# meyer-lab/cmtf-pls

Measured on AMD Instinct MI355X. Metric: nipals_iters_per_sec, higher is better.
Workload: dtype f32

## Files before the change

### cmtf_pls_amd/csrc/xcov.hip

```cpp
#include "common.hpp"

namespace cmtfpls {

typedef double d4_t __attribute__((ext_vector_type(4)));

void launch_reduce_rows(const double* part, int nrows, int64_t P, double* out, hipStream_t st);

XcovPlan plan_xcov(int64_t I, int64_t P) {
  XcovPlan p;
  p.col_tiles = (int)((P + 255) / 256);
#ifndef CMTFPLS_XCOV_BLOCKS
#define CMTFPLS_XCOV_BLOCKS 1024
#endif
  int64_t want = (CMTFPLS_XCOV_BLOCKS + p.col_tiles - 1) / p.col_tiles;
  if (want < 1) want = 1;
  int64_t rpb = (I + want - 1) / want;
  rpb = (rpb + 63) / 64 * 64;
  if (rpb < 64) rpb = 64;
  p.rows_per_block = (int)rpb;
  p.row_blocks = (int)((I + rpb - 1) / rpb);
  if (p.row_blocks < 1) p.row_blocks = 1;
  return p;
}

template <typename T, bool MASKED, bool VEC, int MT, bool FAST, bool SSQ = false, bool STATS = false>
__global__ __launch_bounds__(256) void xcov_kernel(const T* __restrict__ X, int64_t I, int64_t P,
                                                  const double* __restrict__ Y, int ldy, int M,
                                                  double* __restrict__ part, int rows_per_block,
                                                  const double* __restrict__ mean = nullptr, double* __restrict__ ssq_part = nullptr) {
  const int lane = threadIdx.x & 63, wv = threadIdx.x >> 6;
  const int kq = lane >> 4, nn = lane & 15;
  const int64_t cb = ((int64_t)blockIdx.x * 4 + wv) * 64;
  if (cb >= P) {
    if (SSQ && lane == 0) ssq_part[((int64_t)blockIdx.y * gridDim.x + blockIdx.x) * 4 + wv] = 0.0;
    return;
  }
  const int64_t c = cb + 4 * nn;
  const int64_t r0 = (int64_t)blockIdx.y * rows_per_block;
  const int64_t r1 = (r0 + rows_per_block < I) ? r0 + rows_per_block : I;
  using XV = Pack<T, 4>;
  d4_t acc[MT][4];
#pragma unroll
  for (int mt = 0; mt < MT; ++mt)
#pragma unroll
    for (int e = 0; e < 4; ++e) acc[mt][e] = d4_t{0.0, 0.0, 0.0, 0.0};
  bool mok[MT];
#pragma unroll
  for (int mt = 0; mt < MT; ++mt) mok[mt] = (mt * 16 + nn) < M;

#ifndef CMTFPLS_XCOV_UN
#define CMTFPLS_XCOV_UN 4
#endif
  constexpr int UN = CMTFPLS_XCOV_UN;
  const int64_t cc = (c < P) ? c : (VEC ? P - 4 : P - 1);
  int ycol[MT];
#pragma unroll
  for (int mt = 0; mt < MT; ++mt) ycol[mt] = mok[mt] ? mt * 16 + nn : M - 1;
  double mu[SSQ ? 4 : 1], ssq = 0.0;
  double cs[STATS ? 4 : 1] = {}, cq[STATS ? 4 : 1] = {};
  if constexpr (SSQ) {
#pragma unroll
    for (int e = 0; e < 4; ++e) mu[e] = mean[(c + e < P) ? c + e : P - 1];
  }

  auto load_stage = [&](XV (&x)[UN], double (&a)[UN][MT], int64_t r) {
#pragma unroll
    for (int s = 0; s < UN; ++s) {
      const int64_t row = r + 4 * s + kq;
      const int64_t rowc = (FAST || row < r1) ? row : r1 - 1;
      if (VEC) {
        x[s] = ld_stream(reinterpret_cast<const XV*>(X + rowc * P + cc));
      } else {
#pragma unroll
        for (int e = 0; e < 4; ++e) x[s].e[e] = X[rowc * P + ((cc + e < P) ? cc + e : P - 1)];
      }
#pragma unroll
      for (int mt = 0; mt < MT; ++mt) a[s][mt] = Y[rowc * ldy + ycol[mt]];
    }
  };
  auto mma_stage = [&](const XV (&x)[UN], const double (&a)[UN][MT], int64_t r) {
#pragma unroll
    for (int s = 0; s < UN; ++s) {
      const bool rok = FAST || (r + 4 * s + kq) < r1;
#pragma unroll
      for (int e = 0; e < 4; ++e) {
        T xv = x[s].e[e];
        if (MASKED) xv = (xv == xv) ? xv : (T)0;
        const double b = (FAST || (rok && c + e < P)) ? (double)xv : 0.0;
        if constexpr (SSQ) {
          const double dv = (FAST || (rok && c + e < P)) ? b - mu[e] : 0.0;
          ssq = fma(dv, dv, ssq);
        }
        if constexpr (STATS) {
          cs[e] += b;
          cq[e] = fma(b, b, cq[e]);
        }
#pragma unroll
        for (int mt = 0; mt < MT; ++mt)
          acc[mt][e] = __builtin_amdgcn_mfma_f64_16x16x4f64((FAST || (rok && mok[mt])) ? a[s][mt] : 0.0, b, acc[mt][e], 0, 0, 0);
      }
    }
  };

  XV xa[UN], xb[UN];
  double aa[UN][MT], ab[UN][MT];
  load_stage(xa, aa, r0);
  for (int64_t r = r0; r < r1; r += 8 * UN) {
    load_stage(xb, ab, r + 4 * UN);
    mma_stage(xa, aa, r);
    load_stage(xa, aa, (FAST && r + 8 * UN >= r1) ? r : r + 8 * UN);
    mma_stage(xb, ab, r + 4 * UN);
  }
  if constexpr (SSQ) {
    ssq = wave_sum(ssq);
    if (lane == 0) ssq_part[((int64_t)blockIdx.y * gridDim.x + blockIdx.x) * 4 + wv] = ssq;
  }
  if constexpr (STATS) {
    double* srow = ssq_part + (int64_t)blockIdx.y * 2 * P;
#pragma unroll
    for (int e = 0; e < 4; ++e) {
      double v = cs[e], w = cq[e];
      v += __shfl_xor(v, 16, kWave);
      v += __shfl_xor(v, 32, kWave);
      w += __shfl_xor(w, 16, kWave);
      w += __shfl_xor(w, 32, kWave);
      if (kq == 0 && c + e < P) { srow[c + e] = v; srow[P + c + e] = w; }
    }
  }
#pragma unroll
  for (int mt = 0; mt < MT; ++mt)
#pragma unroll
    for (int g = 0; g < 4; ++g) {
      const int m = mt * 16 + kq + 4 * g;
      if (m < M) {
        double* dst = part + ((int64_t)blockIdx.y * M + m) * P + c;
#pragma unroll
        for (int e = 0; e < 4; ++e)
          if (c + e < P) dst[e] = acc[mt][e][g];
      }
    }
}

template <typename T, int MT, bool FAST>
__global__ __launch_bounds__(256) void xcov_deflate_kernel(T* __restrict__ X, int64_t I, int64_t P, int B,
                                                          const double* __restrict__ Y, int ldy, int M,
                                                          double* __restrict__ part, int rows_per_block,
                                                          const double* __restrict__ t, const double* __restrict__ wA,
                                                          const double* __restrict__ wB, double* __restrict__ ssq_part) {
  const int lane = threadIdx.x & 63, wv = threadIdx.x >> 6;
  const int kq = lane >> 4, nn = lane & 15;
  const int64_t cb = ((int64_t)blockIdx.x * 4 + wv) * 64;
  if (cb >= P) {
    if (lane == 0) ssq_part[((int64_t)blockIdx.y * gridDim.x + blockIdx.x) * 4 + wv] = 0.0;
    return;
  }
  const int64_t c = cb + 4 * nn;
  const int64_t r0 = (int64_t)blockIdx.y * rows_per_block;
  const int64_t r1 = (r0 + rows_per_block < I) ? r0 + rows_per_block : I;
  using XV = Pack<T, 4>;
  d4_t acc[MT][4];
#pragma unroll
  for (int mt = 0; mt < MT; ++mt)
#pragma unroll
    for (int e = 0; e < 4; ++e) acc[mt][e] = d4_t{0.0, 0.0, 0.0, 0.0};
  bool mok[MT];
#pragma unroll
  for (int mt = 0; mt < MT; ++mt) mok[mt] = (mt * 16 + nn) < M;
  constexpr int UN = CMTFPLS_XCOV_UN;
  const bool cok = c < P;
  const int64_t cc = cok ? c : P - 4;
  int ycol[MT];
#pragma unroll
  for (int mt = 0; mt < MT; ++mt) ycol[mt] = mok[mt] ? mt * 16 + nn : M - 1;
  double wa[4], wb[4], ssq = 0.0;
#pragma unroll
  for (int e = 0; e < 4; ++e) {
    wa[e] = wA[(cc + e) / B];
    wb[e] = wB[(cc + e) % B];
  }

  auto load_stage = [&](XV (&x)[UN], double (&a)[UN][MT], double (&ts)[UN], int64_t r) {
#pragma unroll
    for (int s = 0; s < UN; ++s) {
      const int64_t row = r + 4 * s + kq;
      const int64_t rowc = (FAST || row < r1) ? row : r1 - 1;
      x[s] = ld_stream(reinterpret_cast<const XV*>(X + rowc * P + cc));
      ts[s] = t[rowc];
#pragma unroll
      for (int mt = 0; mt < MT; ++mt) a[s][mt] = Y[rowc * ldy + ycol[mt]];
    }
  };
  auto mma_stage = [&](XV (&x)[UN], const double (&a)[UN][MT], const double (&ts)[UN], int64_t r) {
#pragma unroll
    for (int s = 0; s < UN; ++s) {
      const int64_t row = r + 4 * s + kq;
      const bool rok = FAST || row < r1;
      const bool ok = rok && (FAST || cok);
#pragma unroll
      for (int e = 0; e < 4; ++e) {
        const double tw = ts[s] * wa[e];
        const T nv = (T)fma(-tw, wb[e], (double)x[s].e[e]);
        x[s].e[e] = nv;
        const double b = (ok && nv == nv) ? (double)nv : 0.0;
        ssq = fma(b, b, ssq);
#pragma unroll
        for (int mt = 0; mt < MT; ++mt)
          acc[mt][e] = __builtin_amdgcn_mfma_f64_16x16x4f64((FAST || (rok && mok[mt])) ? a[s][mt] : 0.0, b, acc[mt][e], 0, 0, 0);
      }
      if (ok) st_stream(reinterpret_cast<XV*>(X + row * P + c), x[s]);
    }
  };

  XV xa[UN], xb[UN];
  double aa[UN][MT], ab[UN][MT], ta[UN], tb[UN];
  load_stage(xa, aa, ta, r0);
  for (int64_t r = r0; r < r1; r += 8 * UN) {
    load_stage(xb, ab, tb, r + 4 * UN);
    mma_stage(xa, aa, ta, r);
    load_stage(xa, aa, ta, (r + 8 * UN >= r1) ? r : r + 8 * UN);
    mma_stage(xb, ab, tb, r + 4 * UN);
  }
  ssq = wave_sum(ssq);
  if (lane == 0) ssq_part[((int64_t)blockIdx.y * gridDim.x + blockIdx.x) * 4 + wv] = ssq;
#pragma unroll
  for (int mt = 0; mt < MT; ++mt)
#pragma unroll
    for (int g = 0; g < 4; ++g) {
      const int m = mt * 16 + kq + 4 * g;
      if (m < M) {
        double* dst = part + ((int64_t)blockIdx.y * M + m) * P + c;
#pragma unroll
        for (int e = 0; e < 4; ++e)
          if (c + e < P) dst[e] = acc[mt][e][g];
      }
    }
}

__global__ __launch_bounds__(256) void quadform_kernel(const double* __restrict__ G, int M, const double* __restrict__ q,
                                                      const double* __restrict__ q_old, double* __restrict__ out) {
  __shared__ double red[16];
  double s = 0.0;
  for (int idx = threadIdx.x; idx < M * M; idx += 256) {
    const int i = idx / M, j = idx - i * M;
    s = fma((q[i] - q_old[i]) * G[idx], (q[j] - q_old[j]), s);
  }
  s = block_sum(s, red);
  if (threadIdx.x == 0) out[0] = s;
}

static size_t xcov_ssq_extra(const XcovPlan& p) { return ((size_t)p.row_blocks * p.col_tiles * 4 * sizeof(double) + 255) / 256 * 256; }

template <typename T>
static int run_xcov_tile(const T* X, int64_t I, int64_t P, const double* Y, int ldy, int M, double* S, int masked,
                         void* ws, size_t ws_bytes, hipStream_t st, const double* mean = nullptr, double* ssq_out = nullptr,
                         double* stats_out = nullptr) {
  const XcovPlan p = plan_xcov(I, P);
  const bool with_ssq = ssq_out != nullptr, with_stats = stats_out != nullptr;
  if (with_ssq && (masked || !mean)) { set_error("xcov_ssq: needs the column means and a block without missing values"); return CMTFPLS_EINVAL; }
  if (with_stats && (masked || with_ssq)) { set_error("xcov_stats: a block without missing values, no second norm"); return CMTFPLS_EINVAL; }
  const size_t need = (size_t)p.row_blocks * M * P * sizeof(double) + (with_ssq ? xcov_ssq_extra(p) : 0) +
                      (with_stats ? (size_t)p.row_blocks * 2 * P * sizeof(double) : 0);
  if (!ws || ws_bytes < need) { set_error("xcov: workspace too small"); return CMTFPLS_EWORKSPACE; }
  const bool vec = (P % 4 == 0) && ((reinterpret_cast<uintptr_t>(X) & (4 * sizeof(T) - 1)) == 0);
  const int mt = (M + 15) / 16;
  double* part = static_cast<double*>(ws);
  const dim3 grid(p.col_tiles, p.row_blocks), block(256);
  const bool fast = vec && (P % 256 == 0) && (M % 16 == 0) && (M / 16 != 3) && (I % p.rows_per_block == 0) &&
                    (p.rows_per_block % (8 * 4) == 0);
  double* ssq_part = (with_ssq || with_stats) ? reinterpret_cast<double*>(static_cast<char*>(ws) + (size_t)p.row_blocks * M * P * sizeof(double)) : nullptr;
#define XL(MSK, VC, MTT, FS) hipLaunchKernelGGL((xcov_kernel<T, MSK, VC, MTT, FS>), grid, block, 0, st, X, I, P, Y, ldy, M, part, p.rows_per_block, (const double*)nullptr, (double*)nullptr)
#define XS(VC, MTT, FS) hipLaunchKernelGGL((xcov_kernel<T, false, VC, MTT, FS, true>), grid, block, 0, st, X, I, P, Y, ldy, M, part, p.rows_per_block, mean, ssq_part)
#define XM(MSK, VC, FS) do { if (mt == 1) XL(MSK, VC, 1, FS); else if (mt == 2) XL(MSK, VC, 2, FS); else XL(MSK, VC, 4, FS); } while (0)
#define XQ(VC, FS) do { if (mt == 1) XS(VC, 1, FS); else if (mt == 2) XS(VC, 2, FS); else XS(VC, 4, FS); } while (0)
#define XT1(VC, MTT, FS) hipLaunchKernelGGL((xcov_kernel<T, false, VC, MTT, FS, false, true>), grid, block, 0, st, X, I, P, Y, ldy, M, part, p.rows_per_block, (const double*)nullptr, ssq_part)
#define XT(VC, FS) do { if (mt == 1) XT1(VC, 1, FS); else if (mt == 2) XT1(VC, 2, FS); else XT1(VC, 4, FS); } while (0)
  if (with_stats)  { if (fast) XT(true, true); else if (vec) XT(true, false); else XT(false, false); }
  else if (with_ssq) { if (fast) XQ(true, true); else if (vec) XQ(true, false); else XQ(false, false); }
  else if (masked) { if (fast) XM(true, true, true); else if (vec) XM(true, true, false); else XM(true, false, false); }
  else             { if (fast) XM(false, true, true); else if (vec) XM(false, true, false); else XM(false, false, false); }
#undef XT
#undef XT1
#undef XQ
#undef XM
#undef XS
#undef XL
  launch_reduce_rows(part, p.row_blocks, (int64_t)M * P, S, st);
  if (with_stats) launch_reduce_rows(ssq_part, p.row_blocks, 2 * P, stats_out, st);
  int rc = check_launch("xcov");
  if (rc == CMTFPLS_OK && with_ssq) rc = cmtfpls_sum_f64(ssq_part, (int64_t)p.row_blocks * p.col_tiles * 4, ssq_out, st);
  return rc;
}

template <typename T>
static int run_xcov(const T* X, int64_t I, int64_t P, const double* Y, int ldy, int M, double* S, int masked,
                    void* ws, size_t ws_bytes, hipStream_t st, const double* mean = nullptr, double* ssq_out = nullptr) {
  if (!X || !Y || !S || I <= 0 || P <= 0 || M <= 0 || ldy < M) { set_error("xcov: bad argument"); return CMTFPLS_EINVAL; }
  for (int lo = 0; lo < M; lo += kXcovMaxResponses) {
    const int mt = (M - lo < kXcovMaxResponses) ? M - lo : kXcovMaxResponses;
    const int rc = run_xcov_tile<T>(X, I, P, Y + lo, ldy, mt, S + (int64_t)lo * P, masked, ws, ws_bytes, st, mean, lo == 0 ? ssq_out : nullptr);
    if (rc != CMTFPLS_OK) return rc;
  }
  return CMTFPLS_OK;
}

template <typename T>
static int run_xcov_deflate(T* X, int64_t I, int A, int B, const double* Y, int ldy, int M, const double* t, const double* wA,
                            const double* wB, double* S, double* ssq, void* ws, size_t ws_bytes, hipStream_t st) {
  if (!X || !Y || !S || !t || !wA || !wB || !ssq || I <= 0 || A <= 0 || B <= 0 || M <= 0 || ldy < M) {
    set_error("xcov_deflate: bad argument");
    return CMTFPLS_EINVAL;
  }
  const int64_t P = (int64_t)A * B;
  if (M > 64 || (P % 4) != 0 || (reinterpret_cast<uintptr_t>(X) & (4 * sizeof(T) - 1)) != 0) {
    set_error("xcov_deflate: M > 64 or rows that are not whole 4-element vectors; deflate, then xcov");
    return CMTFPLS_EUNSUPPORTED;
  }
  const XcovPlan p = plan_xcov(I, P);
  const size_t need = (size_t)p.row_blocks * M * P * sizeof(double) + xcov_ssq_extra(p);
  if (!ws || ws_bytes < need) { set_error("xcov_deflate: workspace too small"); return CMTFPLS_EWORKSPACE; }
  const int mt = (M + 15) / 16;
  double* part = static_cast<double*>(ws);
  double* ssq_part = reinterpret_cast<double*>(static_cast<char*>(ws) + (size_t)p.row_blocks * M * P * sizeof(double));
  const dim3 grid(p.col_tiles, p.row_blocks), block(256);
  const bool fast = (P % 256 == 0) && (M % 16 == 0) && (M / 16 != 3) && (I % p.rows_per_block == 0) && (p.rows_per_block % (8 * 4) == 0);
#define XD(MTT, FS) hipLaunchKernelGGL((xcov_deflate_kernel<T, MTT, FS>), grid, block, 0, st, X, I, P, B, Y, ldy, M, part, p.rows_per_block, t, wA, wB, ssq_part)
  if (fast) { if (mt == 1) XD(1, true); else if (mt == 2) XD(2, true); else XD(4, true); }
  else      { if (mt == 1) XD(1, false); else if (mt == 2) XD(2, false); else XD(4, false); }
#undef XD
  launch_reduce_rows(part, p.row_blocks, (int64_t)M * P, S, st);
  int rc = check_launch("xcov_deflate");
  if (rc == CMTFPLS_OK) rc = cmtfpls_sum_f64(ssq_part, (int64_t)p.row_blocks * p.col_tiles * 4, ssq, st);
  return rc;
}

}

using namespace cmtfpls;

extern "C" {

size_t cmtfpls_xcov_workspace_bytes(int64_t I, int64_t P, int M) {
  if (I <= 0 || P <= 0 || M <= 0) return 0;
  const XcovPlan p = plan_xcov(I, P);
  if (M > kXcovMaxResponses) M = kXcovMaxResponses;
  return (size_t)p.row_blocks * M * P * sizeof(double);
}
int cmtfpls_xcov_f32(const float* X, int64_t I, int64_t P, const double* Y, int ldy, int M, double* S, int masked,
                     void* ws, size_t ws_bytes, void* stream) {
  return run_xcov<float>(X, I, P, Y, ldy, M, S, masked, ws, ws_bytes, (hipStream_t)stream);
}
int cmtfpls_xcov_f64(const double* X, int64_t I, int64_t P, const double* Y, int ldy, int M, double* S, int masked,
                     void* ws, size_t ws_bytes, void* stream) {
  return run_xcov<double>(X, I, P, Y, ldy, M, S, masked, ws, ws_bytes, (hipStream_t)stream);
}
size_t cmtfpls_xcov_ssq_workspace_bytes(int64_t I, int64_t P, int M) {
  if (I <= 0 || P <= 0 || M <= 0) return 0;
  const XcovPlan p = plan_xcov(I, P);
  if (M > kXcovMaxResponses) M = kXcovMaxResponses;
  return (size_t)p.row_blocks * M * P * sizeof(double) + xcov_ssq_extra(p);
}
int cmtfpls_xcov_ssq_f32(const float* X, int64_t I, int64_t P, const double* Y, int ldy, int M, double* S, const double* mean,
                         double* ssq, void* ws, size_t ws_bytes, void* stream) {
  if (!mean || !ssq) { set_error("xcov_ssq: bad argument"); return CMTFPLS_EINVAL; }
  return run_xcov<float>(X, I, P, Y, ldy, M, S, 0, ws, ws_bytes, (hipStream_t)stream, mean, ssq);
}
int cmtfpls_xcov_ssq_f64(const double* X, int64_t I, int64_t P, const double* Y, int ldy, int M, double* S, const double* mean,
                         double* ssq, void* ws, size_t ws_bytes, void* stream) {
  if (!mean || !ssq) { set_error("xcov_ssq: bad argument"); return CMTFPLS_EINVAL; }
  return run_xcov<double>(X, I, P, Y, ldy, M, S, 0, ws, ws_bytes, (hipStream_t)stream, mean, ssq);
}
size_t cmtfpls_xcov_stats_workspace_bytes(int64_t I, int64_t P, int M) {
  if (I <= 0 || P <= 0 || M <= 0 || M > kXcovMaxResponses) return 0;
  const XcovPlan p = plan_xcov(I, P);
  return (size_t)p.row_blocks * ((size_t)M + 2) * P * sizeof(double);
}
int cmtfpls_xcov_stats_f32(const float* X, int64_t I, int64_t P, const double* Y, int ldy, int M, double* S, double* stats,
                           void* ws, size_t ws_bytes, void* stream) {
  if (!X || !Y || !S || !stats || I <= 0 || P <= 0 || M <= 0 || ldy < M) { set_error("xcov_stats: bad argument"); return CMTFPLS_EINVAL; }
  if (M > kXcovMaxResponses) { set_error("xcov_stats: more than 64 responses; use colstats + xcov"); return CMTFPLS_EUNSUPPORTED; }
  return run_xcov_tile<float>(X, I, P, Y, ldy, M, S, 0, ws, ws_bytes, (hipStream_t)stream, nullptr, nullptr, stats);
}
int cmtfpls_xcov_stats_f64(const double* X, int64_t I, int64_t P, const double* Y, int ldy, int M, double* S, double* stats,
                           void* ws, size_t ws_bytes, void* stream) {
  if (!X || !Y || !S || !stats || I <= 0 || P <= 0 || M <= 0 || ldy < M) { set_error("xcov_stats: bad argument"); return CMTFPLS_EINVAL; }
  if (M > kXcovMaxResponses) { set_error("xcov_stats: more than 64 responses; use colstats + xcov"); return CMTFPLS_EUNSUPPORTED; }
  return run_xcov_tile<double>(X, I, P, Y, ldy, M, S, 0, ws, ws_bytes, (hipStream_t)stream, nullptr, nullptr, stats);
}
int cmtfpls_xcov_deflate_f32(float* X, int64_t I, int A, int B, const double* Y, int ldy, int M, const double* t, const double* wA,
                             const double* wB, double* S, double* ssq, void* ws, size_t ws_bytes, void* stream) {
  return run_xcov_deflate<float>(X, I, A, B, Y, ldy, M, t, wA, wB, S, ssq, ws, ws_bytes, (hipStream_t)stream);
}
int cmtfpls_xcov_deflate_f64(double* X, int64_t I, int A, int B, const double* Y, int ldy, int M, const double* t, const double* wA,
                             const double* wB, double* S, double* ssq, void* ws, size_t ws_bytes, void* stream) {
  return run_xcov_deflate<double>(X, I, A, B, Y, ldy, M, t, wA, wB, S, ssq, ws, ws_bytes, (hipStream_t)stream);
}
int cmtfpls_quadform_f64(const double* G, int M, const double* q, const double* q_old, double* out, void* stream) {
  if (!G || !q || !q_old || !out || M <= 0) { set_error("quadform: bad argument"); return CMTFPLS_EINVAL; }
  hipLaunchKernelGGL(quadform_kernel, dim3(1), dim3(256), 0, (hipStream_t)stream, G, M, q, q_old, out);
  return check_launch("quadform");
}

}
```

Before: 762.1.

## Have each wave cover multiple 64-column groups in xcov kernels to reuse Y loads

Result: no change. 761.8 (-0.0%).

```diff
diff --git a/cmtf_pls_amd/csrc/xcov.hip b/cmtf_pls_amd/csrc/xcov.hip
--- a/cmtf_pls_amd/csrc/xcov.hip
+++ b/cmtf_pls_amd/csrc/xcov.hip
@@ -23,86 +23,111 @@
   return p;
 }
 
-template <typename T, bool MASKED, bool VEC, int MT, bool FAST, bool SSQ = false, bool STATS = false>
+constexpr int xcov_groups(int MT) { return MT <= 2 ? 2 : 1; }
+#ifndef CMTFPLS_XCOV_UN
+#define CMTFPLS_XCOV_UN 4
+#endif
+
+template <int G>
+__device__ __forceinline__ void xcov_zero_slots(double* ssq_part, int64_t g0, int ngroups, int lane) {
+  if (lane < G && g0 + lane < ngroups) ssq_part[(int64_t)blockIdx.y * ngroups + g0 + lane] = 0.0;
+}
+
+template <typename T, bool MASKED, bool VEC, int MT, int G, bool FAST, bool SSQ = false, bool STATS = false>
 __global__ __launch_bounds__(256) void xcov_kernel(const T* __restrict__ X, int64_t I, int64_t P,
                                                   const double* __restrict__ Y, int ldy, int M,
-                                                  double* __restrict__ part, int rows_per_block,
+                                                  double* __restrict__ part, int rows_per_block, int ngroups,
                                                   const double* __restrict__ mean = nullptr, double* __restrict__ ssq_part = nullptr) {
   const int lane = threadIdx.x & 63, wv = threadIdx.x >> 6;
   const int kq = lane >> 4, nn = lane & 15;
-  const int64_t cb = ((int64_t)blockIdx.x * 4 + wv) * 64;
+  const int64_t g0 = ((int64_t)blockIdx.x * 4 + wv) * G;
+  const int64_t cb = g0 * 64;
   if (cb >= P) {
-    if (SSQ && lane == 0) ssq_part[((int64_t)blockIdx.y * gridDim.x + blockIdx.x) * 4 + wv] = 0.0;
+    if (SSQ) xcov_zero_slots<G>(ssq_part, g0, ngroups, lane);
     return;
   }
-  const int64_t c = cb + 4 * nn;
   const int64_t r0 = (int64_t)blockIdx.y * rows_per_block;
   const int64_t r1 = (r0 + rows_per_block < I) ? r0 + rows_per_block : I;
   using XV = Pack<T, 4>;
-  d4_t acc[MT][4];
-#pragma unroll
-  for (int mt = 0; mt < MT; ++mt)
-#pragma unroll
-    for (int e = 0; e < 4; ++e) acc[mt][e] = d4_t{0.0, 0.0, 0.0, 0.0};
+  d4_t acc[G][MT][4];
+#pragma unroll
+  for (int g = 0; g < G; ++g)
+#pragma unroll
+    for (int mt = 0; mt < MT; ++mt)
+#pragma unroll
+      for (int e = 0; e < 4; ++e) acc[g][mt][e] = d4_t{0.0, 0.0, 0.0, 0.0};
   bool mok[MT];
 #pragma unroll
   for (int mt = 0; mt < MT; ++mt) mok[mt] = (mt * 16 + nn) < M;
 
-#ifndef CMTFPLS_XCOV_UN
-#define CMTFPLS_XCOV_UN 4
-#endif
   constexpr int UN = CMTFPLS_XCOV_UN;
-  const int64_t cc = (c < P) ? c : (VEC ? P - 4 : P - 1);
+  int64_t c[G], cc[G];
+#pragma unroll
+  for (int g = 0; g < G; ++g) {
+    c[g] = cb + 64 * g + 4 * nn;
+    cc[g] = (c[g] < P) ? c[g] : (VEC ? P - 4 : P - 1);
+  }
   int ycol[MT];
 #pragma unroll
   for (int mt = 0; mt < MT; ++mt) ycol[mt] = mok[mt] ? mt * 16 + nn : M - 1;
-  double mu[SSQ ? 4 : 1], ssq = 0.0;
-  double cs[STATS ? 4 : 1] = {}, cq[STATS ? 4 : 1] = {};
+  double mu[SSQ ? G : 1][4], ssq[G] = {};
+  double cs[STATS ? G : 1][4] = {}, cq[STATS ? G : 1][4] = {};
   if constexpr (SSQ) {
 #pragma unroll
-    for (int e = 0; e < 4; ++e) mu[e] = mean[(c + e < P) ? c + e : P - 1];
-  }
-
-  auto load_stage = [&](XV (&x)[UN], double (&a)[UN][MT], int64_t r) {
+    for (int g = 0; g < G; ++g)
+#pragma unroll
+      for (int e = 0; e < 4; ++e) mu[g][e] = mean[(c[g] + e < P) ? c[g] + e : P - 1];
+  }
+
+  auto load_stage = [&](XV (&x)[UN][G], double (&a)[UN][MT], int64_t r) {
 #pragma unroll
     for (int s = 0; s < UN; ++s) {
       const int64_t row = r + 4 * s + kq;
       const int64_t rowc = (FAST || row < r1) ? row : r1 - 1;
-      if (VEC) {
-        x[s] = ld_stream(reinterpret_cast<const XV*>(X + rowc * P + cc));
-      } else {
-#pragma unroll
-        for (int e = 0; e < 4; ++e) x[s].e[e] = X[rowc * P + ((cc + e < P) ? cc + e : P - 1)];
+#pragma unroll
+      for (int g = 0; g < G; ++g) {
+        if (VEC) {
+          x[s][g] = ld_stream(reinterpret_cast<const XV*>(X + rowc * P + cc[g]));
+        } else {
+#pragma unroll
+          for (int e = 0; e < 4; ++e) x[s][g].e[e] = X[rowc * P + ((cc[g] + e < P) ? cc[g] + e : P - 1)];
+        }
       }
 #pragma unroll
       for (int mt = 0; mt < MT; ++mt) a[s][mt] = Y[rowc * ldy + ycol[mt]];
     }
   };
-  auto mma_stage = [&](const XV (&x)[UN], const double (&a)[UN][MT], int64_t r) {
+  auto mma_stage = [&](const XV (&x)[UN][G], const double (&a)[UN][MT], int64_t r) {
 #pragma unroll
     for (int s = 0; s < UN; ++s) {
       const bool rok = FAST || (r + 4 * s + kq) < r1;
-#pragma unroll
-      for (int e = 0; e < 4; ++e) {
-        T xv = x[s].e[e];
-        if (MASKED) xv = (xv == xv) ? xv : (T)0;
-        const double b = (FAST || (rok && c + e < P)) ? (double)xv : 0.0;
-        if constexpr (SSQ) {
-          const double dv = (FAST || (rok && c + e < P)) ? b - mu[e] : 0.0;
-          ssq = fma(dv, dv, ssq);
+      double am[MT];
+#pragma unroll
+      for (int mt = 0; mt < MT; ++mt) am[mt] = (FAST || (rok && mok[mt])) ? a[s][mt] : 0.0;
+#pragma unroll
+      for (int g = 0; g < G; ++g) {
+#pragma unroll
+        for (int e = 0; e < 4; ++e) {
+          T xv = x[s][g].e[e];
+          if (MASKED) xv = (xv == xv) ? xv : (T)0;
+          const double b = (FAST || (rok && c[g] + e < P)) ? (double)xv : 0.0;
+          if constexpr (SSQ) {
+            const double dv = (FAST || (rok && c[g] + e < P)) ? b - mu[g][e] : 0.0;
+            ssq[g] = fma(dv, dv, ssq[g]);
+          }
+          if constexpr (STATS) {
+            cs[g][e] += b;
+            cq[g][e] = fma(b, b, cq[g][e]);
+          }
+#pragma unroll
+          for (int mt = 0; mt < MT; ++mt)
+            acc[g][mt][e] = __builtin_amdgcn_mfma_f64_16x16x4f64(am[mt], b, acc[g][mt][e], 0, 0, 0);
         }
-        if constexpr (STATS) {
-          cs[e] += b;
-          cq[e] = fma(b, b, cq[e]);
-        }
-#pragma unroll
-        for (int mt = 0; mt < MT; ++mt)
-          acc[mt][e] = __builtin_amdgcn_mfma_f64_16x16x4f64((FAST || (rok && mok[mt])) ? a[s][mt] : 0.0, b, acc[mt][e], 0, 0, 0);
       }
     }
   };
 
-  XV xa[UN], xb[UN];
+  XV xa[UN][G], xb[UN][G];
   double aa[UN][MT], ab[UN][MT];
   load_stage(xa, aa, r0);
   for (int64_t r = r0; r < r1; r += 8 * UN) {
@@ -112,106 +137,128 @@
     mma_stage(xb, ab, r + 4 * UN);
   }
   if constexpr (SSQ) {
-    ssq = wave_sum(ssq);
-    if (lane == 0) ssq_part[((int64_t)blockIdx.y * gridDim.x + blockIdx.x) * 4 + wv] = ssq;
+#pragma unroll
+    for (int g = 0; g < G; ++g) {
+      const double v = wave_sum(ssq[g]);
+      if (lane == 0 && g0 + g < ngroups) ssq_part[(int64_t)blockIdx.y * ngroups + g0 + g] = v;
+    }
   }
   if constexpr (STATS) {
     double* srow = ssq_part + (int64_t)blockIdx.y * 2 * P;
 #pragma unroll
-    for (int e = 0; e < 4; ++e) {
-      double v = cs[e], w = cq[e];
-      v += __shfl_xor(v, 16, kWave);
-      v += __shfl_xor(v, 32, kWave);
-      w += __shfl_xor(w, 16, kWave);
-      w += __shfl_xor(w, 32, kWave);
-      if (kq == 0 && c + e < P) { srow[c + e] = v; srow[P + c + e] = w; }
-    }
-  }
-#pragma unroll
-  for (int mt = 0; mt < MT; ++mt)
-#pragma unroll
-    for (int g = 0; g < 4; ++g) {
-      const int m = mt * 16 + kq + 4 * g;
-      if (m < M) {
-        double* dst = part + ((int64_t)blockIdx.y * M + m) * P + c;
-#pragma unroll
-        for (int e = 0; e < 4; ++e)
-          if (c + e < P) dst[e] = acc[mt][e][g];
-      }
-    }
-}
-
-template <typename T, int MT, bool FAST>
+    for (int g = 0; g < G; ++g)
+#pragma unroll
+      for (int e = 0; e < 4; ++e) {
+        double v = cs[g][e], w = cq[g][e];
+        v += __shfl_xor(v, 16, kWave);
+        v += __shfl_xor(v, 32, kWave);
+        w += __shfl_xor(w, 16, kWave);
+        w += __shfl_xor(w, 32, kWave);
+        if (kq == 0 && c[g] + e < P) { srow[c[g] + e] = v; srow[P + c[g] + e] = w; }
+      }
+  }
+#pragma unroll
+  for (int g = 0; g < G; ++g)
+#pragma unroll
+    for (int mt = 0; mt < MT; ++mt)
+#pragma unroll
+      for (int j = 0; j < 4; ++j) {
+        const int m = mt * 16 + kq + 4 * j;
+        if (m < M) {
+          double* dst = part + ((int64_t)blockIdx.y * M + m) * P + c[g];
+#pragma unroll
+          for (int e = 0; e < 4; ++e)
+            if (c[g] + e < P) dst[e] = acc[g][mt][e][j];
+        }
+      }
+}
+
+template <typename T, int MT, int G, bool FAST>
 __global__ __launch_bounds__(256) void xcov_deflate_kernel(T* __restrict__ X, int64_t I, int64_t P, int B,
                                                           const double* __restrict__ Y, int ldy, int M,
-                                                          double* __restrict__ part, int rows_per_block,
+                                                          double* __restrict__ part, int rows_per_block, int ngroups,
                                                           const double* __restrict__ t, const double* __restrict__ wA,
                                                           const double* __restrict__ wB, double* __restrict__ ssq_part) {
   const int lane = threadIdx.x & 63, wv = threadIdx.x >> 6;
   const int kq = lane >> 4, nn = lane & 15;
-  const int64_t cb = ((int64_t)blockIdx.x * 4 + wv) * 64;
+  const int64_t g0 = ((int64_t)blockIdx.x * 4 + wv) * G;
+  const int64_t cb = g0 * 64;
   if (cb >= P) {
-    if (lane == 0) ssq_part[((int64_t)blockIdx.y * gridDim.x + blockIdx.x) * 4 + wv] = 0.0;
+    xcov_zero_slots<G>(ssq_part, g0, ngroups, lane);
     return;
   }
-  const int64_t c = cb + 4 * nn;
   const int64_t r0 = (int64_t)blockIdx.y * rows_per_block;
   const int64_t r1 = (r0 + rows_per_block < I) ? r0 + rows_per_block : I;
   using XV = Pack<T, 4>;
-  d4_t acc[MT][4];
-#pragma unroll
-  for (int mt = 0; mt < MT; ++mt)
-#pragma unroll
-    for (int e = 0; e < 4; ++e) acc[mt][e] = d4_t{0.0, 0.0, 0.0, 0.0};
+  d4_t acc[G][MT][4];
+#pragma unroll
+  for (int g = 0; g < G; ++g)
+#pragma unroll
+    for (int mt = 0; mt < MT; ++mt)
+#pragma unroll
+      for (int e = 0; e < 4; ++e) acc[g][mt][e] = d4_t{0.0, 0.0, 0.0, 0.0};
   bool mok[MT];
 #pragma unroll
   for (int mt = 0; mt < MT; ++mt) mok[mt] = (mt * 16 + nn) < M;
   constexpr int UN = CMTFPLS_XCOV_UN;
-  const bool cok = c < P;
-  const int64_t cc = cok ? c : P - 4;
+  int64_t c[G], cc[G];
+  bool cok[G];
   int ycol[MT];
 #pragma unroll
   for (int mt = 0; mt < MT; ++mt) ycol[mt] = mok[mt] ? mt * 16 + nn : M - 1;
-  double wa[4], wb[4], ssq = 0.0;
-#pragma unroll
-  for (int e = 0; e < 4; ++e) {
-    wa[e] = wA[(cc + e) / B];
-    wb[e] = wB[(cc + e) % B];
-  }
-
-  auto load_stage = [&](XV (&x)[UN], double (&a)[UN][MT], double (&ts)[UN], int64_t r) {
+  double wa[G][4], wb[G][4], ssq[G] = {};
+#pragma unroll
+  for (int g = 0; g < G; ++g) {
+    c[g] = cb + 64 * g + 4 * nn;
+    cok[g] = c[g] < P;
+    cc[g] = cok[g] ? c[g] : P - 4;
+#pragma unroll
+    for (int e = 0; e < 4; ++e) {
+      wa[g][e] = wA[(cc[g] + e) / B];
+      wb[g][e] = wB[(cc[g] + e) % B];
+    }
+  }
+
+  auto load_stage = [&](XV (&x)[UN][G], double (&a)[UN][MT], double (&ts)[UN], int64_t r) {
 #pragma unroll
     for (int s = 0; s < UN; ++s) {
       const int64_t row = r + 4 * s + kq;
       const int64_t rowc = (FAST || row < r1) ? row : r1 - 1;
-      x[s] = ld_stream(reinterpret_cast<const XV*>(X + rowc * P + cc));
+#pragma unroll
+      for (int g = 0; g < G; ++g) x[s][g] = ld_stream(reinterpret_cast<const XV*>(X + rowc * P + cc[g]));
       ts[s] = t[rowc];
 #pragma unroll
       for (int mt = 0; mt < MT; ++mt) a[s][mt] = Y[rowc * ldy + ycol[mt]];
     }
   };
-  auto mma_stage = [&](XV (&x)[UN], const double (&a)[UN][MT], const double (&ts)[UN], int64_t r) {
+  auto mma_stage = [&](XV (&x)[UN][G], const double (&a)[UN][MT], const double (&ts)[UN], int64_t r) {
 #pragma unroll
     for (int s = 0; s < UN; ++s) {
       const int64_t row = r + 4 * s + kq;
       const bool rok = FAST || row < r1;
-      const bool ok = rok && (FAST || cok);
-#pragma unroll
-      for (int e = 0; e < 4; ++e) {
-        const double tw = ts[s] * wa[e];
-        const T nv = (T)fma(-tw, wb[e], (double)x[s].e[e]);
-        x[s].e[e] = nv;
-        const double b = (ok && nv == nv) ? (double)nv : 0.0;
-        ssq = fma(b, b, ssq);
-#pragma unroll
-        for (int mt = 0; mt < MT; ++mt)
-          acc[mt][e] = __builtin_amdgcn_mfma_f64_16x16x4f64((FAST || (rok && mok[mt])) ? a[s][mt] : 0.0, b, acc[mt][e], 0, 0, 0);
-      }
-      if (ok) st_stream(reinterpret_cast<XV*>(X + row * P + c), x[s]);
+      double am[MT];
+#pragma unroll
+      for (int mt = 0; mt < MT; ++mt) am[mt] = (FAST || (rok && mok[mt])) ? a[s][mt] : 0.0;
+#pragma unroll
+      for (int g = 0; g < G; ++g) {
+        const bool ok = rok && (FAST || cok[g]);
+#pragma unroll
+        for (int e = 0; e < 4; ++e) {
+          const double tw = ts[s] * wa[g][e];
+          const T nv = (T)fma(-tw, wb[g][e], (double)x[s][g].e[e]);
+          x[s][g].e[e] = nv;
+          const double b = (ok && nv == nv) ? (double)nv : 0.0;
+          ssq[g] = fma(b, b, ssq[g]);
+#pragma unroll
+          for (int mt = 0; mt < MT; ++mt)
+            acc[g][mt][e] = __builtin_amdgcn_mfma_f64_16x16x4f64(am[mt], b, acc[g][mt][e], 0, 0, 0);
+        }
+        if (ok) st_stream(reinterpret_cast<XV*>(X + row * P + c[g]), x[s][g]);
+      }
     }
   };
 
-  XV xa[UN], xb[UN];
+  XV xa[UN][G], xb[UN][G];
   double aa[UN][MT], ab[UN][MT], ta[UN], tb[UN];
   load_stage(xa, aa, ta, r0);
   for (int64_t r = r0; r < r1; r += 8 * UN) {
@@ -220,20 +267,25 @@
     load_stage(xa, aa, ta, (r + 8 * UN >= r1) ? r : r + 8 * UN);
     mma_stage(xb, ab, tb, r + 4 * UN);
   }
-  ssq = wave_sum(ssq);
-  if (lane == 0) ssq_part[((int64_t)blockIdx.y * gridDim.x + blockIdx.x) * 4 + wv] = ssq;
-#pragma unroll
-  for (int mt = 0; mt < MT; ++mt)
-#pragma unroll
-    for (int g = 0; g < 4; ++g) {
-      const int m = mt * 16 + kq + 4 * g;
-      if (m < M) {
-        double* dst = part + ((int64_t)blockIdx.y * M + m) * P + c;
-#pragma unroll
-        for (int e = 0; e < 4; ++e)
-          if (c + e < P) dst[e] = acc[mt][e][g];
-      }
-    }
+#pragma unroll
+  for (int g = 0; g < G; ++g) {
+    const double v = wave_sum(ssq[g]);
+    if (lane == 0 && g0 + g < ngroups) ssq_part[(int64_t)blockIdx.y * ngroups + g0 + g] = v;
+  }
+#pragma unroll
+  for (int g = 0; g < G; ++g)
+#pragma unroll
+    for (int mt = 0; mt < MT; ++mt)
+#pragma unroll
+      for (int j = 0; j < 4; ++j) {
+        const int m = mt * 16 + kq + 4 * j;
+        if (m < M) {
+          double* dst = part + ((int64_t)blockIdx.y * M + m) * P + c[g];
+#pragma unroll
+          for (int e = 0; e < 4; ++e)
+            if (c[g] + e < P) dst[e] = acc[g][mt][e][j];
+        }
+      }
 }
 
 __global__ __launch_bounds__(256) void quadform_kernel(const double* __restrict__ G, int M, const double* __restrict__ q,
@@ -249,6 +301,32 @@
 }
 
 static size_t xcov_ssq_extra(const XcovPlan& p) { return ((size_t)p.row_blocks * p.col_tiles * 4 * sizeof(double) + 255) / 256 * 256; }
+
+template <typename T>
+struct XcovArgs {
+  const T* X; int64_t I, P; const double* Y; int ldy, M; double* part; const XcovPlan* plan; const double* mean; double* ssq_part;
+  bool vec, fast; hipStream_t st;
+};
+
+template <typename T, bool MSK, bool SSQ, bool STATS, int MT>
+static void launch_xcov(const XcovArgs<T>& a) {
+  constexpr int G = xcov_groups(MT);
+  const XcovPlan& p = *a.plan;
+  const dim3 grid((p.col_tiles + G - 1) / G, p.row_blocks), block(256);
+  const int ngroups = 4 * p.col_tiles;
+#define XL(VC, FS) hipLaunchKernelGGL((xcov_kernel<T, MSK, VC, MT, G, FS, SSQ, STATS>), grid, block, 0, a.st, a.X, a.I, a.P, a.Y, a.ldy, a.M, \
+                                      a.part, p.rows_per_block, ngroups, a.mean, a.ssq_part)
+  if (a.fast && p.col_tiles % G == 0) XL(true, true);
+  else if (a.vec) XL(true, false);
+  else XL(false, false);
+#undef XL
+}
+template <typename T, bool MSK, bool SSQ, bool STATS>
+static void launch_xcov_mt(const XcovArgs<T>& a, int mt) {
+  if (mt == 1) launch_xcov<T, MSK, SSQ, STATS, 1>(a);
+  else if (mt == 2) launch_xcov<T, MSK, SSQ, STATS, 2>(a);
+  else launch_xcov<T, MSK, SSQ, STATS, 4>(a);
+}
 
 template <typename T>
 static int run_xcov_tile(const T* X, int64_t I, int64_t P, const double* Y, int ldy, int M, double* S, int masked,
@@ -264,26 +342,14 @@
   const bool vec = (P % 4 == 0) && ((reinterpret_cast<uintptr_t>(X) & (4 * sizeof(T) - 1)) == 0);
   const int mt = (M + 15) / 16;
   double* part = static_cast<double*>(ws);
-  const dim3 grid(p.col_tiles, p.row_blocks), block(256);
   const bool fast = vec && (P % 256 == 0) && (M % 16 == 0) && (M / 16 != 3) && (I % p.rows_per_block == 0) &&
                     (p.rows_per_block % (8 * 4) == 0);
   double* ssq_part = (with_ssq || with_stats) ? reinterpret_cast<double*>(static_cast<char*>(ws) + (size_t)p.row_blocks * M * P * sizeof(double)) : nullptr;
-#define XL(MSK, VC, MTT, FS) hipLaunchKernelGGL((xcov_kernel<T, MSK, VC, MTT, FS>), grid, block, 0, st, X, I, P, Y, ldy, M, part, p.rows_per_block, (const double*)nullptr, (double*)nullptr)
-#define XS(VC, MTT, FS) hipLaunchKernelGGL((xcov_kernel<T, false, VC, MTT, FS, true>), grid, block, 0, st, X, I, P, Y, ldy, M, part, p.rows_per_block, mean, ssq_part)
-#define XM(MSK, VC, FS) do { if (mt == 1) XL(MSK, VC, 1, FS); else if (mt == 2) XL(MSK, VC, 2, FS); else XL(MSK, VC, 4, FS); } while (0)
-#define XQ(VC, FS) do { if (mt == 1) XS(VC, 1, FS); else if (mt == 2) XS(VC, 2, FS); else XS(VC, 4, FS); } while (0)
-#define XT1(VC, MTT, FS) hipLaunchKernelGGL((xcov_kernel<T, false, VC, MTT, FS, false, true>), grid, block, 0, st, X, I, P, Y, ldy, M, part, p.rows_per_block, (const double*)nullptr, ssq_part)
-#define XT(VC, FS) do { if (mt == 1) XT1(VC, 1, FS); else if (mt == 2) XT1(VC, 2, FS); else XT1(VC, 4, FS); } while (0)
-  if (with_stats)  { if (fast) XT(true, true); else if (vec) XT(true, false); else XT(false, false); }
-  else if (with_ssq) { if (fast) XQ(true, true); else if (vec) XQ(true, false); else XQ(false, false); }
-  else if (masked) { if (fast) XM(true, true, true); else if (vec) XM(true, true, false); else XM(true, false, false); }
-  else             { if (fast) XM(false, true, true); else if (vec) XM(false, true, false); else XM(false, false, false); }
-#undef XT
-#undef XT1
-#undef XQ
-#undef XM
-#undef XS
-#undef XL
+  const XcovArgs<T> a{X, I, P, Y, ldy, M, part, &p, with_ssq ? mean : nullptr, ssq_part, vec, fast, st};
+  if (with_stats)    launch_xcov_mt<T, false, false, true>(a, mt);
+  else if (with_ssq) launch_xcov_mt<T, false, true, false>(a, mt);
+  else if (masked)   launch_xcov_mt<T, true, false, false>(a, mt);
+  else               launch_xcov_mt<T, false, false, false>(a, mt);
   launch_reduce_rows(part, p.row_blocks, (int64_t)M * P, S, st);
   if (with_stats) launch_reduce_rows(ssq_part, p.row_blocks, 2 * P, stats_out, st);
   int rc = check_launch("xcov");
@@ -304,6 +370,23 @@
 }
 
 template <typename T>
+struct XcovDeflateArgs {
+  T* X; int64_t I, P; int B; const double* Y; int ldy, M; double* part; const XcovPlan* plan; const double *t, *wA, *wB; double* ssq_part;
+  bool fast; hipStream_t st;
+};
+template <typename T, int MT>
+static void launch_xcov_deflate(const XcovDeflateArgs<T>& a) {
+  constexpr int G = xcov_groups(MT);
+  const XcovPlan& p = *a.plan;
+  const dim3 grid((p.col_tiles + G - 1) / G, p.row_blocks), block(256);
+  const int ngroups = 4 * p.col_tiles;
+#define XD(FS) hipLaunchKernelGGL((xcov_deflate_kernel<T, MT, G, FS>), grid, block, 0, a.st, a.X, a.I, a.P, a.B, a.Y, a.ldy, a.M, a.part, \
+                                  p.rows_per_block, ngroups, a.t, a.wA, a.wB, a.ssq_part)
+  if (a.fast && p.col_tiles % G == 0) XD(true); else XD(false);
+#undef XD
+}
+
+template <typename T>
 static int run_xcov_deflate(T* X, int64_t I, int A, int B, const double* Y, int ldy, int M, const double* t, const double* wA,
                             const double* wB, double* S, double* ssq, void* ws, size_t ws_bytes, hipStream_t st) {
   if (!X || !Y || !S || !t || !wA || !wB || !ssq || I <= 0 || A <= 0 || B <= 0 || M <= 0 || ldy < M) {
@@ -321,12 +404,9 @@
   const int mt = (M + 15) / 16;
   double* part = static_cast<double*>(ws);
   double* ssq_part = reinterpret_cast<double*>(static_cast<char*>(ws) + (size_t)p.row_blocks * M * P * sizeof(double));
-  const dim3 grid(p.col_tiles, p.row_blocks), block(256);
   const bool fast = (P % 256 == 0) && (M % 16 == 0) && (M / 16 != 3) && (I % p.rows_per_block == 0) && (p.rows_per_block % (8 * 4) == 0);
-#define XD(MTT, FS) hipLaunchKernelGGL((xcov_deflate_kernel<T, MTT, FS>), grid, block, 0, st, X, I, P, B, Y, ldy, M, part, p.rows_per_block, t, wA, wB, ssq_part)
-  if (fast) { if (mt == 1) XD(1, true); else if (mt == 2) XD(2, true); else XD(4, true); }
-  else      { if (mt == 1) XD(1, false); else if (mt == 2) XD(2, false); else XD(4, false); }
-#undef XD
+  const XcovDeflateArgs<T> a{X, I, P, B, Y, ldy, M, part, &p, t, wA, wB, ssq_part, fast, st};
+  if (mt == 1) launch_xcov_deflate<T, 1>(a); else if (mt == 2) launch_xcov_deflate<T, 2>(a); else launch_xcov_deflate<T, 4>(a);
   launch_reduce_rows(part, p.row_blocks, (int64_t)M * P, S, st);
   int rc = check_launch("xcov_deflate");
   if (rc == CMTFPLS_OK) rc = cmtfpls_sum_f64(ssq_part, (int64_t)p.row_blocks * p.col_tiles * 4, ssq, st);
```
